# chalkydri/chalkydri

Measured on AMD Instinct MI355X. Metric: frames/sec (detect+pose) on 1280x800 batch; HBM GB/s vs roofline, higher is better.
Workload: dtype u8 (threshold/segment/clusters: integer; quad fit/decode/SQPnP: f64)

## Files before the change

chalkydri_amd/csrc/k_quads.hip:

```cpp
#include <stdlib.h>

#include <utility>

#include "ck_internal.h"

namespace {

struct FitArgs {
    const uint8_t *qim; int qw, qh, qstride; size_t qpitch;
    const uint16_t *wimg;
    const uint8_t *im; int w, h, stride; size_t pitch;
    int decimate, refine, max_nmaxima, min_tag_width, normal_ok, reversed_ok;
    double cos_critical, max_mse;
    ck_stage_ws ws;
    int stop_after;
    int guided;
    int list_cap;
    const uint32_t *list;
    const uint32_t *list_count;
    uint32_t *head;
};

struct M6 { long long Mx, My, Mxx, Mxy, Myy, W; };
__device__ __forceinline__ M6 m6_add(M6 a, M6 b) { a.Mx += b.Mx; a.My += b.My; a.Mxx += b.Mxx; a.Mxy += b.Mxy; a.Myy += b.Myy; a.W += b.W; return a; }
// ... 14 lines not shown
    if (inv) frac = (1ull << 30) - frac;
    return ((unsigned long long)oct << 57) | (frac << 26) | ((unsigned long long)x << 13) | (unsigned long long)y;
}
__device__ __forceinline__ uint32_t isqrt_u32(uint32_t v) {
    uint32_t r = (uint32_t)__fsqrt_rn((float)v);
    if (r * r > v) r--;
    if ((r + 1) * (r + 1) <= v) r++;
    return r;
}

__device__ __forceinline__ double f64_of_u52(unsigned long long x) {
    return __longlong_as_double((long long)(0x4330000000000000ull | x)) - 4503599627370496.0;
}

__device__ __forceinline__ void fit_line_m(const M6 &m, int N, double *lineparm, double *err, double *mse) {
    double inv = 1.0 / f64_of_u52((unsigned long long)m.W);
    double Ex = (0.5 * f64_of_u52((unsigned long long)m.Mx)) * inv;
    double Ey = (0.5 * f64_of_u52((unsigned long long)m.My)) * inv;
    double Cxx = (0.25 * f64_of_u52((unsigned long long)m.Mxx)) * inv - Ex * Ex;
    double Cxy = (0.25 * f64_of_u52((unsigned long long)m.Mxy)) * inv - Ex * Ey;
    double Cyy = (0.25 * f64_of_u52((unsigned long long)m.Myy)) * inv - Ey * Ey;
    double d = Cxx - Cyy;
    double q = 4.0 * Cxy;
    double disc = sqrt(d * d + q * Cxy);
    double tr = Cxx + Cyy;
    double eig_small = 0.5 * (tr - disc);
    if (lineparm) {
        lineparm[0] = Ex; lineparm[1] = Ey;
        double eig = 0.5 * (tr + disc);
        double nx1 = Cxx - eig, ny1 = Cxy;
        double M1 = nx1 * nx1 + ny1 * ny1;
        double nx2 = Cxy, ny2 = Cyy - eig;
        double M2 = nx2 * nx2 + ny2 * ny2;
        double nx, ny, M;
        if (M1 > M2) { nx = nx1; ny = ny1; M = M1; } else { nx = nx2; ny = ny2; M = M2; }
        double length = sqrt(M);
        if (length < 1e-12) { lineparm[2] = 0; lineparm[3] = 0; }
        else { lineparm[2] = nx / length; lineparm[3] = ny / length; }
    }
    if (err) *err = (double)N * eig_small;
    if (mse) *mse = eig_small;
}

__device__ const double k_smooth[7] = {0.011108996538242306, 0.1353352832366127, 0.6065306597126334, 1.0,
                                       0.6065306597126334, 0.1353352832366127, 0.011108996538242306};

constexpr int WAIT_VMCNT0 = 0x0F70;
#if defined(__HIP_DEVICE_COMPILE__) && !defined(__GFX9__)
#error "WAIT_VMCNT0 is the gfx9-family encoding of s_waitcnt (this library is written for gfx950): another target needs its own"
#endif
__device__ __forceinline__ void lds_barrier() { asm volatile("s_waitcnt lgkmcnt(0)\n\ts_barrier" ::: "memory"); }
__device__ __forceinline__ void wave_sync() { asm volatile("" ::: "memory"); __builtin_amdgcn_wave_barrier(); asm volatile("" ::: "memory"); }

template <int NTH>
struct Block {
    static constexpr int NW = NTH / 64;
    __device__ __forceinline__ static void sync() { if constexpr (NTH == 64) wave_sync(); else __syncthreads(); }
    __device__ static long long scan_incl(long long v, long long *scratch, long long *total) {
        const int tid = threadIdx.x, lane = tid & 63, wv = tid >> 6;
        long long x = (long long)wave_scan_u64((unsigned long long)v);
        if (NW > 1) {
            if (lane == 63) scratch[wv] = x;
            __syncthreads();
            long long base = 0, tot = 0;
            for (int k = 0; k < NW; k++) { long long t = scratch[k]; if (k < wv) base += t; tot += t; }
            x += base;
            if (total) *total = tot;
            __syncthreads();
        } else if (total) *total = __shfl(x, 63, 64);
        return x;
    }
    __device__ static int reduce_min(int v, int *scratch) {
        const int tid = threadIdx.x, lane = tid & 63, wv = tid >> 6;
        v = wave_min_i32(v);
        if (NW > 1) {
            if (lane == 0) scratch[wv] = v;
            __syncthreads();
            int r = scratch[0];
            for (int k = 1; k < NW; k++) r = min(r, scratch[k]);
            __syncthreads();
            return r;
        }
        return v;
    }
    __device__ static long long reduce_add(long long v, long long *scratch) {
        const int tid = threadIdx.x, lane = tid & 63, wv = tid >> 6;
        {
            const unsigned long long t = wave_scan_u64((unsigned long long)v);
            v = (long long)(((unsigned long long)(uint32_t)__builtin_amdgcn_readlane((int)(t >> 32), 63) << 32) |
                            (uint32_t)__builtin_amdgcn_readlane((int)(uint32_t)t, 63));
        }
        if (NW > 1) {
            if (lane == 0) scratch[wv] = v;
            __syncthreads();
            long long r = 0;
            for (int k = 0; k < NW; k++) r += scratch[k];
            __syncthreads();
            return r;
        }
        return v;
    }
    __device__ static void scan_incl_3x64_3x32(unsigned long long a[3], uint32_t b[3], long long *scratch) {
        const int tid = threadIdx.x, lane = tid & 63, wv = tid >> 6;
#pragma unroll
        for (int q = 0; q < 3; q++) { a[q] = wave_scan_u64(a[q]); b[q] = wave_scan_u32(b[q]); }
        if (NW > 1) {
            unsigned long long *s64 = reinterpret_cast<unsigned long long *>(scratch);
            uint32_t *s32 = reinterpret_cast<uint32_t *>(scratch + 3 * NW);
            if (lane == 63)
#pragma unroll
                for (int q = 0; q < 3; q++) { s64[q * NW + wv] = a[q]; s32[q * NW + wv] = b[q]; }
            __syncthreads();
#pragma unroll
            for (int q = 0; q < 3; q++) {
                unsigned long long ba = 0;
                uint32_t bb = 0;
                for (int k = 0; k < wv; k++) { ba += s64[q * NW + k]; bb += s32[q * NW + k]; }
                a[q] += ba; b[q] += bb;
            }
            __syncthreads();
        }
    }
    __device__ static void reduce_min4(int v[4], int *scratch ) {
        const int tid = threadIdx.x, lane = tid & 63, wv = tid >> 6;
#pragma unroll
        for (int q = 0; q < 4; q++) v[q] = wave_min_i32(v[q]);
        if (NW > 1) {
            if (lane == 0)
#pragma unroll
                for (int q = 0; q < 4; q++) scratch[q * NW + wv] = v[q];
            __syncthreads();
#pragma unroll
            for (int q = 0; q < 4; q++) {
                int r = scratch[q * NW];
                for (int k = 1; k < NW; k++) r = min(r, scratch[q * NW + k]);
                v[q] = r;
            }
            __syncthreads();
        }
    }
    __device__ static int scan_flag(int flag, int *scratch , int *total) {
        const int tid = threadIdx.x, lane = tid & 63, wv = tid >> 6;
        const unsigned long long bal = __ballot(flag != 0);
        int incl = __popcll(bal & ((2ull << lane) - 1ull));
        int tot = __popcll(bal);
        if (NW > 1) {
            if (lane == 0) scratch[wv] = tot;
            __syncthreads();
            int base = 0;
            tot = 0;
            for (int k = 0; k < NW; k++) { int t = scratch[k]; if (k < wv) base += t; tot += t; }
            incl += base;
            __syncthreads();
        }
        *total = tot;
        return incl;
    }
};

#ifdef CK_FIT_PROFILE
__device__ unsigned long long g_fit_prof[3][16];
#define PROF_DECL unsigned long long prof_t0 = __builtin_readcyclecounter(); const int prof_cls = (CAP == 512) ? 0 : (CAP <= 4096 ? 1 : 2)
#define PROF(k) do { unsigned long long t_ = __builtin_readcyclecounter(); if (tid == 0) atomicAdd(&g_fit_prof[prof_cls][k], t_ - prof_t0); prof_t0 = t_; } while (0)
#else
#define PROF_DECL
#define PROF(k)
#endif

constexpr int HALO = 24;
constexpr int MAXSEL = 12;

struct PairFit { double err, mse, nx, ny; };

struct PairTable {
    uint8_t v[MAXSEL * (MAXSEL - 1) / 2];
    constexpr PairTable() : v() {
        int k = 0;
        for (int b = 1; b < MAXSEL; b++)
            for (int a = 0; a < b; a++) v[k++] = (uint8_t)((a << 4) | b);
    }
};
__device__ const PairTable g_pair_table{};
struct ComboTable {
    uint16_t v[495];
    constexpr ComboTable() : v() {
        int k = 0;
        for (int m3 = 3; m3 < MAXSEL; m3++)
            for (int m2 = 2; m2 < m3; m2++)
                for (int m1 = 1; m1 < m2; m1++)
                    for (int m0 = 0; m0 < m1; m0++) v[k++] = (uint16_t)((m0 << 12) | (m1 << 8) | (m2 << 4) | m3);
    }
};
__device__ const ComboTable g_combo_table{};

constexpr int INV_N = 41 * 362 + 1;
struct InvTable {
    double v[INV_N];
    constexpr InvTable() : v() {
        v[0] = __builtin_huge_val();
        for (int n = 1; n < INV_N; n++) v[n] = 1.0 / (double)n;
    }
};
__device__ const InvTable g_inv_table{};

__device__ __forceinline__ int wrap_index(int i, int sz) {
    if (i < 0) i += sz;
    if (i >= sz) i -= sz;
    return i;
}
__device__ __forceinline__ M6 moments_of(uint32_t xy, uint32_t Wt) {
    const uint32_t X = (xy >> 13) + 1, Y = (xy & 0x1FFF) + 1;
    const uint32_t wx = Wt * X, wy = Wt * Y;
    M6 m;
    m.Mx = (long long)wx; m.My = (long long)wy;
    m.Mxx = (long long)((unsigned long long)wx * X); m.Mxy = (long long)((unsigned long long)wx * Y); m.Myy = (long long)((unsigned long long)wy * Y);
    m.W = (long long)Wt;
    return m;
}


template <int NTH, int EPL, int K, int J>
__device__ __forceinline__ void sort_stage(unsigned long long (&k)[EPL], unsigned long long *buf) {
    const int t = threadIdx.x;
    if constexpr (J < EPL) {
#pragma unroll
        for (int e = 0; e < EPL; e++) {
            if ((e & J) == 0) {
                const int i = t * EPL + e;
                const bool up = (i & K) == 0;
                unsigned long long a = k[e], b = k[e | J];
                const bool sw = (a > b) == up;
                k[e] = sw ? b : a; k[e | J] = sw ? a : b;
            }
        }
    } else {
        constexpr int TJ = J / EPL;
        const bool lower = (t & TJ) == 0;
        if constexpr (TJ < 64) {
#pragma unroll
            for (int e = 0; e < EPL; e++) {
                const int i = t * EPL + e;
                const bool up = (i & K) == 0;
                unsigned long long mine = k[e];
                unsigned long long other = __shfl_xor(mine, TJ, 64);
                const bool take_min = (lower == up);
                k[e] = take_min ? (mine < other ? mine : other) : (mine > other ? mine : other);
            }
        } else {
            __syncthreads();
#pragma unroll
            for (int e = 0; e < EPL; e++) buf[t * EPL + e] = k[e];
            __syncthreads();
#pragma unroll
            for (int e = 0; e < EPL; e++) {
                const int i = t * EPL + e;
                const bool up = (i & K) == 0;
                unsigned long long mine = k[e];
                unsigned long long other = buf[(t ^ TJ) * EPL + e];
                const bool take_min = (lower == up);
                k[e] = take_min ? (mine < other ? mine : other) : (mine > other ? mine : other);
            }
        }
    }
}
template <int NTH, int EPL, int K, int J>
struct SortJ {
    __device__ __forceinline__ static void run(unsigned long long (&k)[EPL], unsigned long long *buf) {
        sort_stage<NTH, EPL, K, J>(k, buf);
        if constexpr (J > 1) SortJ<NTH, EPL, K, J / 2>::run(k, buf);
    }
};
template <int NTH, int EPL, int K>
struct SortK {
    __device__ __forceinline__ static void run(unsigned long long (&k)[EPL], unsigned long long *buf) {
        SortJ<NTH, EPL, K, K / 2>::run(k, buf);
        if constexpr (K < NTH * EPL) SortK<NTH, EPL, K * 2>::run(k, buf);
    }
};
template <int NTH, int EPL>
__device__ __forceinline__ void sort_registers(unsigned long long (&k)[EPL], unsigned long long *buf) {
    SortK<NTH, EPL, 2>::run(k, buf);
}

template <int NTH, int EPL>
__device__ __forceinline__ long long keys_sort(unsigned long long *sKeys, long long *sScratch, int sz0, int xmin, int xmax, int ymin, int ymax,
                                               int normal_ok, int reversed_ok, bool do_sort = true) {
    using B = Block<NTH>;
    const int tid = threadIdx.x;
    unsigned long long kreg[EPL];
    long long dot = 0;
#pragma unroll
    for (int e = 0; e < EPL; e++) {
        int i = tid * EPL + e;
        unsigned long long key = ~0ull;
        if (i < sz0) {
            unsigned long long raw = sKeys[i];
            int px = (int)(raw & 0xFFFF), py = (int)((raw >> 16) & 0xFFFF);
            int pgx = (int)(signed char)((raw >> 32) & 0xFF), pgy = (int)(signed char)((raw >> 40) & 0xFF);
            const int dx = 4 * px - 2 * (xmin + xmax) - 1, dy = 4 * py - 2 * (ymin + ymax) + 1;
            dot += (long long)(dx * pgx + dy * pgy);
            key = angle_key(px, py, xmin, xmax, ymin, ymax);
        }
        kreg[e] = key;
    }
    dot = B::reduce_add(dot, sScratch);
    if (do_sort && ((dot < 0) ? reversed_ok : normal_ok)) {
        sort_registers<NTH, EPL>(kreg, sKeys);
        __syncthreads();
#pragma unroll
        for (int e = 0; e < EPL; e++) sKeys[tid * EPL + e] = kreg[e];
    }
    return dot;
}

constexpr int BUCKET_LIMIT = 32;
template <int NTH, int EPLS>
__device__ __forceinline__ long long keys_bucket_sort(unsigned long long *sKeys, uint32_t *hist , long long *sScratch, int sz0,
                                                      int xmin, int xmax, int ymin, int ymax, int normal_ok, int reversed_ok, bool do_sort,
                                                      bool *done) {
    using B = Block<NTH>;
    const int tid = threadIdx.x;
    int n2 = NTH;
    while (n2 < sz0) n2 <<= 1;
    int nb = n2 > 2048 ? 2048 : n2;
    const int lgq = (31 - __clz(nb)) - 3;
    for (int i = tid; i <= nb; i += NTH) hist[i] = 0;
    unsigned long long kreg[EPLS];
    uint32_t meta[EPLS];
    long long dot = 0;
#pragma unroll
    for (int e = 0; e < EPLS; e++) {
        const int i = tid + e * NTH;
        kreg[e] = 0; meta[e] = 0;
        if (i < sz0) {
            unsigned long long raw = sKeys[i];
            int px = (int)(raw & 0xFFFF), py = (int)((raw >> 16) & 0xFFFF);
            int pgx = (int)(signed char)((raw >> 32) & 0xFF), pgy = (int)(signed char)((raw >> 40) & 0xFF);
            const int dx = 4 * px - 2 * (xmin + xmax) - 1, dy = 4 * py - 2 * (ymin + ymax) + 1;
            dot += (long long)(dx * pgx + dy * pgy);
            kreg[e] = angle_key(px, py, xmin, xmax, ymin, ymax);
        }
    }
    dot = B::reduce_add(dot, sScratch);
    *done = true;
    if (!do_sort || !((dot < 0) ? reversed_ok : normal_ok)) return dot;
    B::sync();
#pragma unroll
    for (int e = 0; e < EPLS; e++) {
        const int i = tid + e * NTH;
        if (i < sz0) {
            const uint32_t oct = (uint32_t)(kreg[e] >> 57), frac = (uint32_t)(kreg[e] >> 26) & 0x7FFFFFFFu;
            uint32_t fb = frac >> (30 - lgq);
            fb = fb > (1u << lgq) - 1 ? (1u << lgq) - 1 : fb;
            const uint32_t b = (oct << lgq) | fb;
            meta[e] = (b << 16) | atomicAdd(&hist[b], 1u);
        }
    }
    B::sync();
    {
        const int per = nb / NTH;
        uint32_t sum = 0, mx = 0;
        for (int q = 0; q < per; q++) { uint32_t c = hist[tid * per + q]; sum += c; mx = mx > c ? mx : c; }
        long long total;
        const long long incl = B::scan_incl((long long)sum, sScratch, &total);
        const int worst = -B::reduce_min(-(int)mx, reinterpret_cast<int *>(sScratch));
        if (worst > BUCKET_LIMIT) { *done = false; B::sync(); return dot; }
        uint32_t run = (uint32_t)(incl - sum);
        for (int q = 0; q < per; q++) { uint32_t c = hist[tid * per + q]; hist[tid * per + q] = run; run += c; }
        if (tid == NTH - 1) hist[nb] = run;
    }
    B::sync();
#pragma unroll
    for (int e = 0; e < EPLS; e++) {
        const int i = tid + e * NTH;
        if (i < sz0) sKeys[hist[meta[e] >> 16] + (meta[e] & 0xFFFFu)] = kreg[e];
    }
    B::sync();
    uint32_t pos[EPLS];
#pragma unroll
    for (int e = 0; e < EPLS; e++) {
        const int i = tid + e * NTH;
        pos[e] = 0;
        if (i < sz0) {
            const uint32_t b = meta[e] >> 16, s0 = hist[b], s1 = hist[b + 1], mine = s0 + (meta[e] & 0xFFFFu);
            const unsigned long long key = kreg[e];
            uint32_t rank = 0;
            for (uint32_t j = s0; j < s1; j++) {
                const unsigned long long o = sKeys[j];
                rank += (o < key || (o == key && j < mine)) ? 1u : 0u;
            }
            pos[e] = s0 + rank;
        }
    }
    B::sync();
#pragma unroll
    for (int e = 0; e < EPLS; e++) {
        const int i = tid + e * NTH;
        if (i < sz0) sKeys[pos[e]] = kreg[e];
    }
    return dot;
}

constexpr int BUCKET_LIMIT_L = 96;
template <int NTH, bool NOLIMIT>
__device__ __forceinline__ long long keys_bucket_sort_global(unsigned long long *sKeys, uint32_t *hist , long long *sScratch,
                                                             unsigned long long *gtmp, int sz0, int xmin, int xmax, int ymin, int ymax,
                                                             int normal_ok, int reversed_ok, bool do_sort, bool *done) {
    using B = Block<NTH>;
    const int tid = threadIdx.x;
    constexpr int nb = 1024, lgq = 7;
    uint32_t *cursor = hist + nb + 1;
    auto bucket_of = [&](unsigned long long key) -> uint32_t {
        const uint32_t oct = (uint32_t)(key >> 57), frac = (uint32_t)(key >> 26) & 0x7FFFFFFFu;
        uint32_t fb = frac >> (30 - lgq);
        fb = fb > (1u << lgq) - 1 ? (1u << lgq) - 1 : fb;
        return (oct << lgq) | fb;
    };
    for (int i = tid; i <= nb; i += NTH) hist[i] = 0;
    __syncthreads();
    long long dot = 0;
// ... 34 lines not shown
        uint32_t rank = 0;
        for (uint32_t k = s0; k < s1; k++) {
            const unsigned long long o = gtmp[k];
            rank += (o < key || (o == key && k < (uint32_t)j)) ? 1u : 0u;
        }
        sKeys[s0 + rank] = key;
    }
    return dot;
}

struct FenceBarrier { __device__ __forceinline__ static void sync() { __syncthreads(); } };
constexpr int RAWP_MAX = 16;
struct Box { int xmin, xmax, ymin, ymax; };

__device__ __forceinline__ uint32_t dq_chunk(uint32_t n_work, uint32_t dqmax) {
    const uint32_t per_wg4 = n_work / (gridDim.x * 4u);
    return per_wg4 < 1u ? 1u : (per_wg4 > dqmax ? dqmax : per_wg4);
}
__device__ __forceinline__ uint32_t dq_guided(uint32_t n_work, uint32_t base, uint32_t dq) {
    const uint32_t g = base < n_work ? (n_work - base) / (gridDim.x * 2u) : 0u;
    return g < 1u ? 1u : (g > dq ? dq : g);
}
template <uint32_t DQMAX, class BAR>
struct ChunkQueue {
    uint32_t n_work, dq, static_total, base, len, dq_next;
    bool first;
    __device__ __forceinline__ explicit ChunkQueue(const FitArgs &a) {
        n_work = min(*a.list_count, (uint32_t)a.list_cap);
        dq = dq_chunk(n_work, DQMAX);
        static_total = gridDim.x * dq;
        base = blockIdx.x * dq; len = dq; dq_next = dq;
        first = true;
    }
    __device__ __forceinline__ bool next(const FitArgs &a, uint32_t *word) {
        if (!first) {
            if (static_total >= n_work) return false;
            BAR::sync();
            if (threadIdx.x == 0) *word = static_total + atomicAdd(a.head, dq_next);
            BAR::sync();
            base = *word;
            len = dq_next;
            if (a.guided) dq_next = dq_guided(n_work, base, dq);
        }
        first = false;
        return base < n_work;
    }
    __device__ __forceinline__ int count() const { return (int)min(len, n_work - base); }
};

template <int NTH, int CAP>
__device__ __forceinline__ Box front_box(const ck_packed_point (&rawp)[CAP / NTH <= RAWP_MAX ? CAP / NTH : 1], const ck_packed_point *pts, int sz0,
                                         unsigned long long *sKeys, int *iscr) {
    constexpr int EPL = CAP / NTH;
    const int tid = threadIdx.x;
    int xmin = 1 << 30, xmax = -(1 << 30), ymin = 1 << 30, ymax = -(1 << 30);
    auto take = [&](int i, ck_packed_point v) {
        const unsigned long long raw = ck_stage_point(v);
        sKeys[i] = raw;
        const int px = (int)(raw & 0xFFFF), py = (int)((raw >> 16) & 0xFFFF);
        xmin = min(xmin, px); xmax = max(xmax, px);
        ymin = min(ymin, py); ymax = max(ymax, py);
    };
    if constexpr (EPL <= RAWP_MAX) {
#pragma unroll
        for (int e = 0; e < EPL; e++) {
            const int i = tid + e * NTH;
            if (i < sz0) take(i, rawp[e]);
        }
    } else {
        for (int i = tid; i < sz0; i += NTH) take(i, pts[i]);
    }
    int bb[4] = {xmin, -xmax, ymin, -ymax};
    Block<NTH>::reduce_min4(bb, iscr);
    return Box{bb[0], -bb[1], bb[2], -bb[3]};
}

template <int NTH, int CAP, bool MLDS, bool GK, class BAR>
__device__ __forceinline__ long long front_sort(unsigned long long *sKeys, uint32_t *hist, long long *sScratch, unsigned long long *scratch8, int sz0,
                                                const Box &b, int normal_ok, int reversed_ok, bool do_sort) {
    constexpr int EPLS = CAP / NTH;
    int n2 = NTH;
    while (n2 < sz0) n2 <<= 1;
    const int epl = n2 / NTH;
    BAR::sync();
    bool sorted = false;
    long long dot;
    if constexpr (MLDS)
        dot = keys_bucket_sort<NTH, EPLS>(sKeys, hist, sScratch, sz0, b.xmin, b.xmax, b.ymin, b.ymax, normal_ok, reversed_ok, do_sort, &sorted);
    else
        dot = keys_bucket_sort_global<NTH, GK>(sKeys, hist, sScratch, scratch8, sz0, b.xmin, b.xmax, b.ymin, b.ymax, normal_ok, reversed_ok, do_sort, &sorted);
    if (sorted || GK) {}
    else if (EPLS >= 32 && epl == 32) dot = keys_sort<NTH, (EPLS >= 32 && !GK ? 32 : 1)>(sKeys, sScratch, sz0, b.xmin, b.xmax, b.ymin, b.ymax, normal_ok, reversed_ok, do_sort);
    else if (EPLS >= 16 && epl == 16) dot = keys_sort<NTH, (EPLS >= 16 && !GK ? 16 : 1)>(sKeys, sScratch, sz0, b.xmin, b.xmax, b.ymin, b.ymax, normal_ok, reversed_ok, do_sort);
    else if (EPLS >= 8 && epl == 8) dot = keys_sort<NTH, (EPLS >= 8 && !GK ? 8 : 1)>(sKeys, sScratch, sz0, b.xmin, b.xmax, b.ymin, b.ymax, normal_ok, reversed_ok, do_sort);
    else if (EPLS >= 4 && epl == 4) dot = keys_sort<NTH, (EPLS >= 4 && !GK ? 4 : 1)>(sKeys, sScratch, sz0, b.xmin, b.xmax, b.ymin, b.ymax, normal_ok, reversed_ok, do_sort);
    else if (EPLS >= 2 && epl == 2) dot = keys_sort<NTH, (EPLS >= 2 && !GK ? 2 : 1)>(sKeys, sScratch, sz0, b.xmin, b.xmax, b.ymin, b.ymax, normal_ok, reversed_ok, do_sort);
    else dot = keys_sort<NTH, 1>(sKeys, sScratch, sz0, b.xmin, b.xmax, b.ymin, b.ymax, normal_ok, reversed_ok, do_sort);
    return dot;
}

template <int NTH, class BAR>
__device__ __forceinline__ int front_pack(unsigned long long *sKeys, int sz0, int *iscr) {
    const int tid = threadIdx.x;
    uint32_t *sXY = reinterpret_cast<uint32_t *>(sKeys);
    int sz = 0;
    for (int base = 0; base < sz0; base += NTH) {
        const int i = base + tid;
        unsigned long long key = 0;
        int keep = 0;
        if (i < sz0) { key = sKeys[i]; keep = (i == 0) || (sKeys[i - 1] != key); }
        int tot = 0;
        const int incl = Block<NTH>::scan_flag(keep, iscr, &tot);
        BAR::sync();
        if (keep) sXY[sz + (int)incl - 1] = (uint32_t)(key & 0x3FFFFFFu);
        sz += (int)tot;
        BAR::sync();
    }
    return sz;
}

template <int NTH, int CAP, int CH, bool MLDS, int WPS, bool GK = false>
__global__ __launch_bounds__(NTH) __attribute__((amdgpu_waves_per_eu(WPS, 8))) void k_fit(FitArgs a) {
    using B = Block<NTH>;
    constexpr int SL = CH + 2 * HALO;
    constexpr int G = (CAP <= 4096) ? 32 : 128;
    constexpr int LPM = (CAP > 4096) ? 32 : (NTH >= MAXSEL * 8) ? 8 : 4;
    static_assert(MAXSEL * LPM <= NTH && CH % G == 0, "one lane group per selected maximum");
    constexpr int NG = CAP / G;
    constexpr int MAXM = MLDS ? (CAP / 2 > 2 * MAXSEL * 6 ? CAP / 2 : 2 * MAXSEL * 6) : 1;
    __shared__ unsigned long long sKeysL[GK ? 1 : CAP];
    const int capr = GK ? a.ws.hcap : CAP;
    unsigned long long *const sKeys = GK ? a.ws.d_hscratch + (size_t)blockIdx.x * 2 * capr : sKeysL;
    constexpr int SPB = 36 * SL > (int)sizeof(PairFit) * MAXSEL * MAXSEL ? 36 * SL : (int)sizeof(PairFit) * MAXSEL * MAXSEL;
    __shared__ __attribute__((aligned(16))) unsigned char sPraw[SPB];
    __shared__ double sErr[SL];
    __shared__ long long sTot[NG + 1][6];
    __shared__ long long sScratch[6 * (NTH / 64) + 2];
    __shared__ double sMaxVal[MAXM];
    __shared__ int sSelIdx[MAXSEL];
    static_assert(MLDS || sizeof(double) * SL >= sizeof(long long) * 2 * MAXSEL * 6, "selected-maxima sums must fit in sErr");
    static_assert(!MLDS || sizeof(double) * MAXM >= sizeof(long long) * 2 * MAXSEL * 6, "selected-maxima sums must fit in sMaxVal");
    long long (*sSelI)[6] = reinterpret_cast<long long (*)[6]>(MLDS ? reinterpret_cast<long long *>(sMaxVal) : reinterpret_cast<long long *>(sErr));
    long long (*sSelE)[6] = sSelI + MAXSEL;
    __shared__ double sRed[NTH / 64 + 1];
    __shared__ int sRedI[NTH / 64 + 1];
    __shared__ uint32_t sWork;
    __shared__ int sNmax, sFlag;
    __shared__ double sLines[4][4];
    __shared__ double sQuad[4][2];
    double (*sRefine)[16][2] = reinterpret_cast<double (*)[16][2]>(sPraw);
    static_assert(SPB >= ((CAP < 2048 ? CAP : 2048) + 1) * 4 || CAP <= 512, "sort histogram must fit in sPraw");
    long long (*sP64)[SL] = reinterpret_cast<long long (*)[SL]>(sPraw);
    uint32_t (*sP32)[SL] = reinterpret_cast<uint32_t (*)[SL]>(sPraw + 24 * SL);
    const int tid = threadIdx.x;
    const ck_stage_ws &ws = a.ws;
    uint32_t *sXY = reinterpret_cast<uint32_t *>(sKeys);
    uint16_t *sW = reinterpret_cast<uint16_t *>(sKeys) + 2 * capr;
    uint16_t *sMaxIdx = reinterpret_cast<uint16_t *>(sKeys) + 3 * capr;

    const uint32_t n_work = min(*a.list_count, (uint32_t)a.list_cap);
    constexpr uint32_t DQMAX = CAP <= 512 ? 16u : (CAP <= 2048 ? 4u : 1u);
    const uint32_t DQ = dq_chunk(n_work, DQMAX);
    const uint32_t static_total = gridDim.x * DQ;
    uint32_t chunk_base = blockIdx.x * DQ, chunk_left = DQ, chunk_len = DQ, dq_next = DQ;
    for (;;) {
        __syncthreads();
        if (chunk_left == 0) {
            if (static_total >= n_work) break;
            if (tid == 0) sWork = static_total + atomicAdd(a.head, dq_next);
            __syncthreads();
            chunk_base = sWork;
            if (chunk_base >= n_work) break;
            chunk_left = chunk_len = dq_next;
            if (a.guided) dq_next = dq_guided(n_work, chunk_base, DQ);
        }
        const uint32_t work = chunk_base + (chunk_len - chunk_left);
        chunk_left--;
        if (work >= n_work) break;
        const uint32_t item = a.list[work];
        const int frame = (int)(item >> 20), ci = (int)(item & 0xFFFFFu);
        const ck_cluster_t cl = ws.d_clusters[(size_t)frame * ws.cluster_cap + ci];
        const ck_packed_point *pts = ws.d_points + (size_t)frame * ws.ext_cap + cl.start;
        unsigned long long *scratch8 = GK ? ws.d_hscratch + (size_t)blockIdx.x * 2 * capr + capr : ws.d_lscratch + (size_t)blockIdx.x * CK_LSCRATCH_PER_WG;
        const int sz0 = (int)cl.count;
        const uint16_t *wq = a.wimg + (size_t)frame * a.qw * a.qh;
        const uint8_t *im = a.im + (size_t)frame * a.pitch;
        if (sz0 > CAP) continue;
        PROF_DECL;
        PROF(15);

        if (a.stop_after == 0) continue;
        constexpr int EPL0 = CAP / NTH;
        ck_packed_point rawp[EPL0 <= RAWP_MAX ? EPL0 : 1];
        if constexpr (EPL0 <= RAWP_MAX) {
#pragma unroll
            for (int e = 0; e < EPL0; e++) { int i = tid + e * NTH; rawp[e] = (i < sz0) ? pts[i] : 0u; }
        }
        int *iscr = reinterpret_cast<int *>(sScratch);
        const Box box = front_box<NTH, CAP>(rawp, pts, sz0, sKeys, iscr);
        if ((box.xmax - box.xmin) * (box.ymax - box.ymin) < a.min_tag_width) continue;
        if (a.stop_after == 10) continue;
        const long long dot = front_sort<NTH, CAP, MLDS, GK, FenceBarrier>(sKeys, reinterpret_cast<uint32_t *>(sPraw), sScratch, scratch8, sz0, box,
                                                                          a.normal_ok, a.reversed_ok, a.stop_after != 11);
        const int reversed = dot < 0;
        PROF(0);
        if (reversed && !a.reversed_ok) continue;
        if (!reversed && !a.normal_ok) continue;
        if (a.stop_after == 1 || a.stop_after == 11) continue;

        __syncthreads();
        PROF(1);
        const int sz = front_pack<NTH, FenceBarrier>(sKeys, sz0, iscr);
        PROF(2);
        if (sz < 24) continue;
        const int ksz = sz / 12 < 20 ? sz / 12 : 20;
        if (ksz < 2) continue;

        if (a.stop_after == 2) continue;
        {
            constexpr int EPL = CAP / NTH;
            if constexpr (EPL <= 16) {
                uint16_t g[EPL];
#pragma unroll
                for (int e = 0; e < EPL; e++) {
                    int i = tid + e * NTH;
                    g[e] = 1;
                    if (i < sz) {
                        uint32_t xy = sXY[i];
                        int x = (int)(xy >> 13), y = (int)(xy & 0x1FFF);
                        int ix = (x + 1) >> 1, iy = (y + 1) >> 1;
                        if (ix >= 0 && ix < a.qw && iy >= 0 && iy < a.qh) g[e] = wq[(size_t)iy * a.qw + ix];
                    }
                }
#pragma unroll
                for (int e = 0; e < EPL; e++) {
                    int i = tid + e * NTH;
                    if (i < sz) sW[i] = g[e];
                }
            } else {
                for (int i = tid; i < sz; i += NTH) {
                    uint32_t xy = sXY[i];
                    int x = (int)(xy >> 13), y = (int)(xy & 0x1FFF);
                    int ix = (x + 1) >> 1, iy = (y + 1) >> 1;
                    sW[i] = (ix >= 0 && ix < a.qw && iy >= 0 && iy < a.qh) ? wq[(size_t)iy * a.qw + ix] : (uint16_t)1;
                }
            }
        }
        double *gval = reinterpret_cast<double *>(scratch8);
        uint32_t *gidx = reinterpret_cast<uint32_t *>(gval + (sz0 + 1) / 2);
        if (tid == 0) { sNmax = 0; sFlag = 0; }
        if (tid < 6) sTot[0][tid] = 0;
        __syncthreads();

        PROF(3);
        if (a.stop_after == 3) continue;
        const int nch = (sz + CH - 1) / CH;
        for (int c = 0; c < nch; c++) {
            const int cbase = c * CH;
            const int chn = min(CH, sz - cbase);
            const int sl = chn + 2 * HALO;
            constexpr int EPT = (SL + NTH - 1) / NTH;
            double carry = 0.0;
            if (c > 0 && tid < 8) carry = sErr[HALO + CH - 4 + tid];
            M6 loc[EPT];
            M6 run = m6_zero();
// ... 439 lines not shown
                        sQuad[j][1] = sLines[i][1] + L0 * A10;
                    }
                }
        }
        if (tid == 0) {
            uint32_t *counters = ws.d_counters + (size_t)frame * CK_CNT_STRIDE;
            uint32_t qi = atomicAdd(&counters[CK_CNT_QUADS], 1u);
            if (qi < (uint32_t)ws.quad_cap) {
                ck_quad_t q;
                for (int i = 0; i < 4; i++) { q.p[i][0] = sQuad[i][0]; q.p[i][1] = sQuad[i][1]; }
                q.reversed_border = reversed; q.rep0 = cl.rep0; q.rep1 = cl.rep1;
                ws.d_quads[(size_t)frame * ws.quad_cap + qi] = q;
            } else atomicOr(&counters[CK_CNT_STATUS], (uint32_t)CK_FRAME_QUADS_OVERFLOW);
        }
        PROF(10);
    }
}

template <int NTH, int CAP, bool MLDS, int WPS, bool GK>
__global__ __launch_bounds__(NTH) __attribute__((amdgpu_waves_per_eu(WPS, 8))) void k_seq(FitArgs a) {
    using B = Block<NTH>;
    constexpr int EPL = CAP / NTH;
    constexpr bool PF = EPL <= RAWP_MAX;
    constexpr int HB = MLDS ? ((CAP < 2048 ? CAP : 2048) + 1) * 4 : 2 * (1024 + 1) * 4;
    __shared__ unsigned long long sKeysL[GK ? 1 : CAP];
    __shared__ __attribute__((aligned(16))) unsigned char sHist[HB];
    __shared__ long long sScratch[6 * (NTH / 64) + 2];
    __shared__ uint32_t sWork;
    __shared__ uint32_t sHItem[64], sHStart[64], sHCount[64];
    const int tid = threadIdx.x;
    const ck_stage_ws &ws = a.ws;
    const int capr = GK ? ws.hcap : CAP;
    unsigned long long *const sKeys = GK ? ws.d_hscratch + (size_t)blockIdx.x * 2 * capr : sKeysL;
    unsigned long long *scratch8 = GK ? ws.d_hscratch + (size_t)blockIdx.x * 2 * capr + capr : ws.d_lscratch + (size_t)blockIdx.x * CK_LSCRATCH_PER_WG;
    uint32_t *sXY = reinterpret_cast<uint32_t *>(sKeys);
    int *iscr = reinterpret_cast<int *>(sScratch);
    constexpr uint32_t DQMAX = CAP <= 512 ? 64u : (CAP <= 1024 ? 32u : (CAP <= 2048 ? 16u : (CAP <= 4096 ? 8u : (CAP <= 8192 ? 4u : 2u))));
    ChunkQueue<DQMAX, B> queue(a);
    while (queue.next(a, &sWork)) {
        const uint32_t chunk_base = queue.base;
        const int len = queue.count();
        B::sync();
        if (tid < len) {
            const uint32_t item = a.list[chunk_base + (uint32_t)tid];
            const ck_cluster_t cl = ws.d_clusters[(size_t)(item >> 20) * ws.cluster_cap + (item & 0xFFFFFu)];
            sHItem[tid] = item; sHStart[tid] = cl.start; sHCount[tid] = cl.count;
        }
        B::sync();
        ck_packed_point nxt[PF ? EPL : 1];
        auto fetch = [&](int k) {
            if constexpr (PF) {
                const uint32_t item = sHItem[k], cnt = sHCount[k];
                const ck_packed_point *p = ws.d_points + (size_t)(item >> 20) * ws.ext_cap + sHStart[k];
#pragma unroll
                for (int e = 0; e < EPL; e++) { const uint32_t i = (uint32_t)(tid + e * NTH); nxt[e] = (i < cnt && cnt <= (uint32_t)CAP) ? p[i] : 0u; }
            }
        };
        fetch(0);
        for (int k = 0; k < len; k++) {
            const uint32_t item = sHItem[k];
            const int frame = (int)(item >> 20), ci = (int)(item & 0xFFFFFu);
            const int sz0 = (int)sHCount[k];
            const ck_packed_point *pts = ws.d_points + (size_t)frame * ws.ext_cap + sHStart[k];
            ck_packed_point rawp[PF ? EPL : 1];
            if constexpr (PF) {
                __builtin_amdgcn_s_waitcnt(WAIT_VMCNT0);
#pragma unroll
                for (int e = 0; e < EPL; e++) rawp[e] = nxt[e];
                if (k + 1 < len) fetch(k + 1);
            }
            B::sync();
            uint32_t *cstate = ws.d_cstate + 2 * ((size_t)frame * ws.cluster_cap + ci);
            if (tid == 0) *cstate = 0u;
            if (sz0 > CAP || sz0 < 1) continue;
            if (a.stop_after == 0) continue;
            const Box box = front_box<NTH, CAP>(rawp, pts, sz0, sKeys, iscr);
            if ((box.xmax - box.xmin) * (box.ymax - box.ymin) < a.min_tag_width) continue;
            if (a.stop_after == 10) continue;
            const long long dot = front_sort<NTH, CAP, MLDS, GK, B>(sKeys, reinterpret_cast<uint32_t *>(sHist), sScratch, scratch8, sz0, box,
                                                                    a.normal_ok, a.reversed_ok, a.stop_after != 11);
            const int reversed = dot < 0;
            if (reversed && !a.reversed_ok) continue;
            if (!reversed && !a.normal_ok) continue;
            if (a.stop_after == 1 || a.stop_after == 11) continue;
            B::sync();
            const int sz = front_pack<NTH, B>(sKeys, sz0, iscr);
            if (sz < 24) continue;
            const int ksz = sz / 12 < 20 ? sz / 12 : 20;
            if (ksz < 2) continue;
            if (a.stop_after == 2) continue;
            if (tid == 0) sWork = atomicAdd(ws.d_counters + (size_t)frame * CK_CNT_STRIDE + CK_CNT_EXT, (uint32_t)(sz + CK_EXT_HALO));
            B::sync();
            const uint32_t es32 = sWork;
            uint32_t *exy = ws.d_ext_xy + (size_t)frame * ws.ext_cap + es32;
            for (int q = tid; q < sz + CK_EXT_HALO; q += NTH) {
                int src = q - CK_EXT_PRE;
                if (src < 0) src += sz;
                if (src < 0) src += sz;
                if (src >= sz) src -= sz;
                exy[q] = sXY[src] | ((uint32_t)ksz << 26);
            }
            if (tid == 0) { cstate[1] = es32; cstate[0] = (uint32_t)sz | (reversed ? 0x80000000u : 0u); }
        }
    }
}

constexpr int KL = 1024, KOFF = 32;
static_assert(CK_SPAN == 960 && KOFF >= CK_EXT_PRE + 3 && KL - KOFF - CK_SPAN >= CK_EXT_POST + 4, "span geometry");
__device__ __forceinline__ void k_chunk_body(const ck_stage_ws &ws, int qw, int qh) {
    __shared__ __attribute__((aligned(16))) unsigned long long sP64[3][KL];
    __shared__ __attribute__((aligned(16))) uint32_t sP32[3][KL];
    __shared__ uint8_t sKsz[KL];
    __shared__ unsigned long long sScan64[3][4];
    __shared__ uint32_t sScan32[3][4];
    __shared__ uint32_t sCnt[16];
    double *sS = reinterpret_cast<double *>(&sP64[0][0]), *sErr = reinterpret_cast<double *>(&sP64[1][0]);
    const int tid = threadIdx.x, lane = tid & 63, wv = tid >> 6;
    const int frame = blockIdx.y;
    const uint32_t *counters = ws.d_counters + (size_t)frame * CK_CNT_STRIDE;
    const uint32_t ext_total = min(counters[CK_CNT_EXT], (uint32_t)ws.ext_cap);
    const uint32_t *xy = ws.d_ext_xy + (size_t)frame * ws.ext_cap;
    uint16_t *w16 = ws.d_ext_w + (size_t)frame * ws.ext_cap;
    const uint16_t *wq = ws.d_wimg + (size_t)frame * qw * qh;
    double *mval = ws.d_maxval + (size_t)frame * (ws.ext_cap / 2);
    uint16_t *mpos = ws.d_maxpos + (size_t)frame * (ws.ext_cap / 2);
    unsigned long long *mmask = ws.d_maxmask + (size_t)frame * (ws.ext_cap / 64);
    uint16_t *mpre = ws.d_maxpre + (size_t)frame * (ws.ext_cap / 64);
    long long *blk = ws.d_blk + (size_t)frame * 6 * (ws.ext_cap / 32);
    auto load_xy = [&](uint32_t s) -> uint4 {
        const long long p0 = (long long)s * CK_SPAN - KOFF + 4 * tid;
        if ((unsigned long long)s * CK_SPAN < ext_total && p0 >= 0 && p0 + 4 <= (long long)ws.ext_cap) return *reinterpret_cast<const uint4 *>(xy + p0);
        return make_uint4(0, 0, 0, 0);
    };
    auto gather_w = [&](uint32_t v) -> uint32_t {
        const int x = (int)((v >> 13) & 0x1FFFu), y = (int)(v & 0x1FFFu);
        const int ix = (x + 1) >> 1, iy = (y + 1) >> 1;
        return (ix < qw && iy < qh) ? (uint32_t)wq[(size_t)iy * qw + ix] : 1u;
    };
    uint4 x4 = load_xy(blockIdx.x);
// ... 903 lines not shown
```

Measured before the change: 18290.

## Keep cluster points in registers through box, bucket sort and dedup pack

Front-end quad fitting no longer writes raw points to LDS in front_box. The register-held points now feed the bucket sort directly, and LDS keys are staged only on the fallback path. The scan and max reductions in the bucket sort are fused into one pass, saving a barrier. The dedup pack becomes a ballot/mbcnt compaction with a small per-wave count table, and loop_tid stops the compiler rematerialising threadIdx. Together these cut LDS traffic and block barriers per cluster, at the cost of register pressure and more template paths.

```diff
diff --git a/chalkydri_amd/csrc/k_quads.hip b/chalkydri_amd/csrc/k_quads.hip
--- a/chalkydri_amd/csrc/k_quads.hip
+++ b/chalkydri_amd/csrc/k_quads.hip
@@ -90,6 +90,8 @@
 __device__ __forceinline__ void lds_barrier() { asm volatile("s_waitcnt lgkmcnt(0)\n\ts_barrier" ::: "memory"); }
 __device__ __forceinline__ void wave_sync() { asm volatile("" ::: "memory"); __builtin_amdgcn_wave_barrier(); asm volatile("" ::: "memory"); }
 
+__device__ __forceinline__ int loop_tid() { int t = threadIdx.x; asm volatile("" : "+v"(t)); return t; }
+
 template <int NTH>
 struct Block {
     static constexpr int NW = NTH / 64;
@@ -159,6 +161,23 @@
             __syncthreads();
         }
     }
+    __device__ static uint32_t scan_incl_max(uint32_t v, uint32_t m, uint32_t *scratch, uint32_t *max_out) {
+        const int tid = threadIdx.x, lane = tid & 63, wv = tid >> 6;
+        uint32_t x = wave_scan_u32(v);
+        uint32_t mx = (uint32_t)-wave_min_i32(-(int)m);
+        if (NW > 1) {
+            if (lane == 63) { scratch[wv] = x; scratch[NW + wv] = mx; }
+            __syncthreads();
+            uint32_t base = 0;
+            mx = scratch[NW];
+            for (int k = 0; k < NW; k++) { const uint32_t t = scratch[k]; if (k < wv) base += t; }
+            for (int k = 1; k < NW; k++) mx = max(mx, scratch[NW + k]);
+            x += base;
+            __syncthreads();
+        }
+        *max_out = mx;
+        return x;
+    }
     __device__ static void reduce_min4(int v[4], int *scratch ) {
         const int tid = threadIdx.x, lane = tid & 63, wv = tid >> 6;
 #pragma unroll
@@ -258,8 +277,7 @@
 
 
 template <int NTH, int EPL, int K, int J>
-__device__ __forceinline__ void sort_stage(unsigned long long (&k)[EPL], unsigned long long *buf) {
-    const int t = threadIdx.x;
+__device__ __forceinline__ void sort_stage(unsigned long long (&k)[EPL], unsigned long long *buf, const int t) {
     if constexpr (J < EPL) {
 #pragma unroll
         for (int e = 0; e < EPL; e++) {
@@ -303,28 +321,28 @@
 }
 template <int NTH, int EPL, int K, int J>
 struct SortJ {
-    __device__ __forceinline__ static void run(unsigned long long (&k)[EPL], unsigned long long *buf) {
-        sort_stage<NTH, EPL, K, J>(k, buf);
-        if constexpr (J > 1) SortJ<NTH, EPL, K, J / 2>::run(k, buf);
+    __device__ __forceinline__ static void run(unsigned long long (&k)[EPL], unsigned long long *buf, const int t) {
+        sort_stage<NTH, EPL, K, J>(k, buf, t);
+        if constexpr (J > 1) SortJ<NTH, EPL, K, J / 2>::run(k, buf, t);
     }
 };
 template <int NTH, int EPL, int K>
 struct SortK {
-    __device__ __forceinline__ static void run(unsigned long long (&k)[EPL], unsigned long long *buf) {
-        SortJ<NTH, EPL, K, K / 2>::run(k, buf);
-        if constexpr (K < NTH * EPL) SortK<NTH, EPL, K * 2>::run(k, buf);
+    __device__ __forceinline__ static void run(unsigned long long (&k)[EPL], unsigned long long *buf, const int t) {
+        SortJ<NTH, EPL, K, K / 2>::run(k, buf, t);
+        if constexpr (K < NTH * EPL) SortK<NTH, EPL, K * 2>::run(k, buf, t);
     }
 };
 template <int NTH, int EPL>
-__device__ __forceinline__ void sort_registers(unsigned long long (&k)[EPL], unsigned long long *buf) {
-    SortK<NTH, EPL, 2>::run(k, buf);
-}
-
-template <int NTH, int EPL>
+__device__ __forceinline__ void sort_registers(unsigned long long (&k)[EPL], unsigned long long *buf, const int t) {
+    SortK<NTH, EPL, 2>::run(k, buf, t);
+}
+
+template <int NTH, int EPL, bool RARE>
 __device__ __forceinline__ long long keys_sort(unsigned long long *sKeys, long long *sScratch, int sz0, int xmin, int xmax, int ymin, int ymax,
                                                int normal_ok, int reversed_ok, bool do_sort = true) {
     using B = Block<NTH>;
-    const int tid = threadIdx.x;
+    const int tid = RARE ? loop_tid() : (int)threadIdx.x;
     unsigned long long kreg[EPL];
     long long dot = 0;
 #pragma unroll
@@ -343,7 +361,7 @@
     }
     dot = B::reduce_add(dot, sScratch);
     if (do_sort && ((dot < 0) ? reversed_ok : normal_ok)) {
-        sort_registers<NTH, EPL>(kreg, sKeys);
+        sort_registers<NTH, EPL>(kreg, sKeys, tid);
         __syncthreads();
 #pragma unroll
         for (int e = 0; e < EPL; e++) sKeys[tid * EPL + e] = kreg[e];
@@ -353,11 +371,11 @@
 
 constexpr int BUCKET_LIMIT = 32;
 template <int NTH, int EPLS>
-__device__ __forceinline__ long long keys_bucket_sort(unsigned long long *sKeys, uint32_t *hist , long long *sScratch, int sz0,
-                                                      int xmin, int xmax, int ymin, int ymax, int normal_ok, int reversed_ok, bool do_sort,
-                                                      bool *done) {
+__device__ __forceinline__ long long keys_bucket_sort(const ck_packed_point (&rawp)[EPLS], unsigned long long *sKeys, uint32_t *hist ,
+                                                      long long *sScratch, int sz0, int xmin, int xmax, int ymin, int ymax, int normal_ok,
+                                                      int reversed_ok, bool do_sort, bool *done) {
     using B = Block<NTH>;
-    const int tid = threadIdx.x;
+    const int tid = loop_tid();
     int n2 = NTH;
     while (n2 < sz0) n2 <<= 1;
     int nb = n2 > 2048 ? 2048 : n2;
@@ -371,7 +389,7 @@
         const int i = tid + e * NTH;
         kreg[e] = 0; meta[e] = 0;
         if (i < sz0) {
-            unsigned long long raw = sKeys[i];
+            const unsigned long long raw = ck_stage_point(rawp[e]);
             int px = (int)(raw & 0xFFFF), py = (int)((raw >> 16) & 0xFFFF);
             int pgx = (int)(signed char)((raw >> 32) & 0xFF), pgy = (int)(signed char)((raw >> 40) & 0xFF);
             const int dx = 4 * px - 2 * (xmin + xmax) - 1, dy = 4 * py - 2 * (ymin + ymax) + 1;
@@ -382,7 +400,7 @@
     dot = B::reduce_add(dot, sScratch);
     *done = true;
     if (!do_sort || !((dot < 0) ? reversed_ok : normal_ok)) return dot;
-    B::sync();
+    if constexpr (B::NW == 1) B::sync();
 #pragma unroll
     for (int e = 0; e < EPLS; e++) {
         const int i = tid + e * NTH;
@@ -397,13 +415,11 @@
     B::sync();
     {
         const int per = nb / NTH;
-        uint32_t sum = 0, mx = 0;
+        uint32_t sum = 0, mx = 0, worst;
         for (int q = 0; q < per; q++) { uint32_t c = hist[tid * per + q]; sum += c; mx = mx > c ? mx : c; }
-        long long total;
-        const long long incl = B::scan_incl((long long)sum, sScratch, &total);
-        const int worst = -B::reduce_min(-(int)mx, reinterpret_cast<int *>(sScratch));
-        if (worst > BUCKET_LIMIT) { *done = false; B::sync(); return dot; }
-        uint32_t run = (uint32_t)(incl - sum);
+        const uint32_t incl = B::scan_incl_max(sum, mx, reinterpret_cast<uint32_t *>(sScratch), &worst);
+        if (worst > (uint32_t)BUCKET_LIMIT) { *done = false; return dot; }
+        uint32_t run = incl - sum;
         for (int q = 0; q < per; q++) { uint32_t c = hist[tid * per + q]; hist[tid * per + q] = run; run += c; }
         if (tid == NTH - 1) hist[nb] = run;
     }
@@ -544,23 +560,19 @@
 __device__ __forceinline__ Box front_box(const ck_packed_point (&rawp)[CAP / NTH <= RAWP_MAX ? CAP / NTH : 1], const ck_packed_point *pts, int sz0,
                                          unsigned long long *sKeys, int *iscr) {
     constexpr int EPL = CAP / NTH;
-    const int tid = threadIdx.x;
+    const int tid = loop_tid();
     int xmin = 1 << 30, xmax = -(1 << 30), ymin = 1 << 30, ymax = -(1 << 30);
-    auto take = [&](int i, ck_packed_point v) {
-        const unsigned long long raw = ck_stage_point(v);
-        sKeys[i] = raw;
-        const int px = (int)(raw & 0xFFFF), py = (int)((raw >> 16) & 0xFFFF);
+    auto take = [&](ck_packed_point v) {
+        const int px = (int)((v >> 16) & 0x1FFFu), py = (int)((v >> 3) & 0x1FFFu);
         xmin = min(xmin, px); xmax = max(xmax, px);
         ymin = min(ymin, py); ymax = max(ymax, py);
     };
     if constexpr (EPL <= RAWP_MAX) {
 #pragma unroll
-        for (int e = 0; e < EPL; e++) {
-            const int i = tid + e * NTH;
-            if (i < sz0) take(i, rawp[e]);
-        }
+        for (int e = 0; e < EPL; e++)
+            if (tid + e * NTH < sz0) take(rawp[e]);
     } else {
-        for (int i = tid; i < sz0; i += NTH) take(i, pts[i]);
+        for (int i = tid; i < sz0; i += NTH) { const ck_packed_point v = pts[i]; sKeys[i] = ck_stage_point(v); take(v); }
     }
     int bb[4] = {xmin, -xmax, ymin, -ymax};
     Block<NTH>::reduce_min4(bb, iscr);
@@ -568,33 +580,91 @@
 }
 
 template <int NTH, int CAP, bool MLDS, bool GK, class BAR>
-__device__ __forceinline__ long long front_sort(unsigned long long *sKeys, uint32_t *hist, long long *sScratch, unsigned long long *scratch8, int sz0,
-                                                const Box &b, int normal_ok, int reversed_ok, bool do_sort) {
+__device__ __forceinline__ long long front_sort(const ck_packed_point (&rawp)[CAP / NTH <= RAWP_MAX ? CAP / NTH : 1], unsigned long long *sKeys,
+                                                uint32_t *hist, long long *sScratch, unsigned long long *scratch8, int sz0, const Box &b,
+                                                int normal_ok, int reversed_ok, bool do_sort) {
     constexpr int EPLS = CAP / NTH;
+    static_assert(MLDS == (EPLS <= RAWP_MAX), "the classes with their keys in registers are the ones with their points in registers");
     int n2 = NTH;
     while (n2 < sz0) n2 <<= 1;
     const int epl = n2 / NTH;
-    BAR::sync();
     bool sorted = false;
     long long dot;
-    if constexpr (MLDS)
-        dot = keys_bucket_sort<NTH, EPLS>(sKeys, hist, sScratch, sz0, b.xmin, b.xmax, b.ymin, b.ymax, normal_ok, reversed_ok, do_sort, &sorted);
-    else
+    if constexpr (MLDS) {
+        dot = keys_bucket_sort<NTH, EPLS>(rawp, sKeys, hist, sScratch, sz0, b.xmin, b.xmax, b.ymin, b.ymax, normal_ok, reversed_ok, do_sort, &sorted);
+        if (!sorted) {
+            const int tid = loop_tid();
+#pragma unroll
+            for (int e = 0; e < EPLS; e++) {
+                const int i = tid + e * NTH;
+                if (i < sz0) sKeys[i] = ck_stage_point(rawp[e]);
+            }
+            BAR::sync();
+        }
+    } else {
+        BAR::sync();
         dot = keys_bucket_sort_global<NTH, GK>(sKeys, hist, sScratch, scratch8, sz0, b.xmin, b.xmax, b.ymin, b.ymax, normal_ok, reversed_ok, do_sort, &sorted);
+    }
     if (sorted || GK) {}
-    else if (EPLS >= 32 && epl == 32) dot = keys_sort<NTH, (EPLS >= 32 && !GK ? 32 : 1)>(sKeys, sScratch, sz0, b.xmin, b.xmax, b.ymin, b.ymax, normal_ok, reversed_ok, do_sort);
-    else if (EPLS >= 16 && epl == 16) dot = keys_sort<NTH, (EPLS >= 16 && !GK ? 16 : 1)>(sKeys, sScratch, sz0, b.xmin, b.xmax, b.ymin, b.ymax, normal_ok, reversed_ok, do_sort);
-    else if (EPLS >= 8 && epl == 8) dot = keys_sort<NTH, (EPLS >= 8 && !GK ? 8 : 1)>(sKeys, sScratch, sz0, b.xmin, b.xmax, b.ymin, b.ymax, normal_ok, reversed_ok, do_sort);
-    else if (EPLS >= 4 && epl == 4) dot = keys_sort<NTH, (EPLS >= 4 && !GK ? 4 : 1)>(sKeys, sScratch, sz0, b.xmin, b.xmax, b.ymin, b.ymax, normal_ok, reversed_ok, do_sort);
-    else if (EPLS >= 2 && epl == 2) dot = keys_sort<NTH, (EPLS >= 2 && !GK ? 2 : 1)>(sKeys, sScratch, sz0, b.xmin, b.xmax, b.ymin, b.ymax, normal_ok, reversed_ok, do_sort);
-    else dot = keys_sort<NTH, 1>(sKeys, sScratch, sz0, b.xmin, b.xmax, b.ymin, b.ymax, normal_ok, reversed_ok, do_sort);
+    else if (EPLS >= 32 && epl == 32) dot = keys_sort<NTH, (EPLS >= 32 && !GK ? 32 : 1), MLDS>(sKeys, sScratch, sz0, b.xmin, b.xmax, b.ymin, b.ymax, normal_ok, reversed_ok, do_sort);
+    else if (EPLS >= 16 && epl == 16) dot = keys_sort<NTH, (EPLS >= 16 && !GK ? 16 : 1), MLDS>(sKeys, sScratch, sz0, b.xmin, b.xmax, b.ymin, b.ymax, normal_ok, reversed_ok, do_sort);
+    else if (EPLS >= 8 && epl == 8) dot = keys_sort<NTH, (EPLS >= 8 && !GK ? 8 : 1), MLDS>(sKeys, sScratch, sz0, b.xmin, b.xmax, b.ymin, b.ymax, normal_ok, reversed_ok, do_sort);
+    else if (EPLS >= 4 && epl == 4) dot = keys_sort<NTH, (EPLS >= 4 && !GK ? 4 : 1), MLDS>(sKeys, sScratch, sz0, b.xmin, b.xmax, b.ymin, b.ymax, normal_ok, reversed_ok, do_sort);
+    else if (EPLS >= 2 && epl == 2) dot = keys_sort<NTH, (EPLS >= 2 && !GK ? 2 : 1), MLDS>(sKeys, sScratch, sz0, b.xmin, b.xmax, b.ymin, b.ymax, normal_ok, reversed_ok, do_sort);
+    else dot = keys_sort<NTH, 1, MLDS>(sKeys, sScratch, sz0, b.xmin, b.xmax, b.ymin, b.ymax, normal_ok, reversed_ok, do_sort);
     return dot;
 }
 
-template <int NTH, class BAR>
-__device__ __forceinline__ int front_pack(unsigned long long *sKeys, int sz0, int *iscr) {
-    const int tid = threadIdx.x;
+template <int NTH, int EPL, class BAR>
+__device__ __forceinline__ int front_pack(unsigned long long *sKeys, int sz0, int *iscr, uint32_t *tbl ) {
+    const int tid = loop_tid();
     uint32_t *sXY = reinterpret_cast<uint32_t *>(sKeys);
+    if constexpr (EPL <= RAWP_MAX) {
+        constexpr int NW = NTH / 64, NT = EPL * NW;
+        static_assert(NT <= 128, "the table is summed by one wave, two entries per lane");
+        const int lane = tid & 63, wv = __builtin_amdgcn_readfirstlane(tid >> 6);
+        uint32_t w[EPL];
+        uint32_t cum[NW == 1 ? EPL : 1], total = 0;
+#pragma unroll
+        for (int e = 0; e < EPL; e++) {
+            const int i = tid + e * NTH;
+            bool keep = false;
+            uint32_t xy = 0;
+            if (i < sz0) {
+                const unsigned long long key = sKeys[i];
+                keep = (i == 0) || (sKeys[i - 1] != key);
+                xy = (uint32_t)(key & 0x3FFFFFFu);
+            }
+            const unsigned long long bal = __ballot(keep);
+            const uint32_t before = __builtin_amdgcn_mbcnt_hi((uint32_t)(bal >> 32), __builtin_amdgcn_mbcnt_lo((uint32_t)bal, 0u));
+            w[e] = keep ? (xy | (before << 26)) : ~0u;
+            if constexpr (NW == 1) { cum[e] = total; total += (uint32_t)__popcll(bal); }
+            else if (lane == 0) tbl[e * NW + wv] = (uint32_t)__popcll(bal);
+        }
+        BAR::sync();
+        if constexpr (NW == 1) {
+#pragma unroll
+            for (int e = 0; e < EPL; e++)
+                if (w[e] != ~0u) sXY[cum[e] + (w[e] >> 26)] = w[e] & 0x3FFFFFFu;
+        } else {
+            const uint32_t c0 = lane < NT ? tbl[lane] : 0u, s0 = wave_scan_u32(c0);
+            const uint32_t x0 = s0 - c0;
+            total = (uint32_t)__builtin_amdgcn_readlane((int)s0, 63);
+            uint32_t x1 = 0;
+            if constexpr (NT > 64) {
+                const uint32_t c1 = lane + 64 < NT ? tbl[lane + 64] : 0u, s1 = wave_scan_u32(c1);
+                x1 = s1 - c1 + total;
+                total += (uint32_t)__builtin_amdgcn_readlane((int)s1, 63);
+            }
+#pragma unroll
+            for (int e = 0; e < EPL; e++) {
+                const uint32_t start = (uint32_t)__builtin_amdgcn_readlane((int)(e * NW < 64 ? x0 : x1), (e * NW + wv) & 63);
+                if (w[e] != ~0u) sXY[start + (w[e] >> 26)] = w[e] & 0x3FFFFFFu;
+            }
+        }
+        BAR::sync();
+        return (int)total;
+    }
     int sz = 0;
     for (int base = 0; base < sz0; base += NTH) {
         const int i = base + tid;
@@ -692,7 +762,7 @@
         const Box box = front_box<NTH, CAP>(rawp, pts, sz0, sKeys, iscr);
         if ((box.xmax - box.xmin) * (box.ymax - box.ymin) < a.min_tag_width) continue;
         if (a.stop_after == 10) continue;
-        const long long dot = front_sort<NTH, CAP, MLDS, GK, FenceBarrier>(sKeys, reinterpret_cast<uint32_t *>(sPraw), sScratch, scratch8, sz0, box,
+        const long long dot = front_sort<NTH, CAP, MLDS, GK, FenceBarrier>(rawp, sKeys, reinterpret_cast<uint32_t *>(sPraw), sScratch, scratch8, sz0, box,
                                                                           a.normal_ok, a.reversed_ok, a.stop_after != 11);
         const int reversed = dot < 0;
         PROF(0);
@@ -702,7 +772,7 @@
 
         __syncthreads();
         PROF(1);
-        const int sz = front_pack<NTH, FenceBarrier>(sKeys, sz0, iscr);
+        const int sz = front_pack<NTH, CAP / NTH, FenceBarrier>(sKeys, sz0, iscr, reinterpret_cast<uint32_t *>(sPraw));
         PROF(2);
         if (sz < 24) continue;
         const int ksz = sz / 12 < 20 ? sz / 12 : 20;
@@ -1248,12 +1318,14 @@
             if constexpr (PF) {
                 const uint32_t item = sHItem[k], cnt = sHCount[k];
                 const ck_packed_point *p = ws.d_points + (size_t)(item >> 20) * ws.ext_cap + sHStart[k];
-#pragma unroll
-                for (int e = 0; e < EPL; e++) { const uint32_t i = (uint32_t)(tid + e * NTH); nxt[e] = (i < cnt && cnt <= (uint32_t)CAP) ? p[i] : 0u; }
+                const int t = loop_tid();
+#pragma unroll
+                for (int e = 0; e < EPL; e++) { const uint32_t i = (uint32_t)(t + e * NTH); nxt[e] = (i < cnt && cnt <= (uint32_t)CAP) ? p[i] : 0u; }
             }
         };
         fetch(0);
         for (int k = 0; k < len; k++) {
+            const int tid = loop_tid();
             const uint32_t item = sHItem[k];
             const int frame = (int)(item >> 20), ci = (int)(item & 0xFFFFFu);
             const int sz0 = (int)sHCount[k];
@@ -1273,14 +1345,14 @@
             const Box box = front_box<NTH, CAP>(rawp, pts, sz0, sKeys, iscr);
             if ((box.xmax - box.xmin) * (box.ymax - box.ymin) < a.min_tag_width) continue;
             if (a.stop_after == 10) continue;
-            const long long dot = front_sort<NTH, CAP, MLDS, GK, B>(sKeys, reinterpret_cast<uint32_t *>(sHist), sScratch, scratch8, sz0, box,
+            const long long dot = front_sort<NTH, CAP, MLDS, GK, B>(rawp, sKeys, reinterpret_cast<uint32_t *>(sHist), sScratch, scratch8, sz0, box,
                                                                     a.normal_ok, a.reversed_ok, a.stop_after != 11);
             const int reversed = dot < 0;
             if (reversed && !a.reversed_ok) continue;
             if (!reversed && !a.normal_ok) continue;
             if (a.stop_after == 1 || a.stop_after == 11) continue;
             B::sync();
-            const int sz = front_pack<NTH, B>(sKeys, sz0, iscr);
+            const int sz = front_pack<NTH, EPL, B>(sKeys, sz0, iscr, reinterpret_cast<uint32_t *>(sHist));
             if (sz < 24) continue;
             const int ksz = sz / 12 < 20 ? sz / 12 : 20;
             if (ksz < 2) continue;
```

Result: faster. 18570, median of 6 (+1.6%).
